# vision-agh/apse_uav

Measured on AMD Instinct MI355X. Metric: 4K UAV frames/sec (whole node), higher is better.
Workload: dtype f32

## Files before the change

apse_uav_amd/csrc/conv1x1_stream.hip:

```cpp
#include "apse_common.h"
#include <stdlib.h>
#include <type_traits>

typedef _Float16 f16x8 __attribute__((ext_vector_type(8)));
typedef unsigned s1_u32x4 __attribute__((ext_vector_type(4)));
__device__ __forceinline__ f32x16 s1_zero16() { return f32x16{0.f, 0.f, 0.f, 0.f, 0.f, 0.f, 0.f, 0.f, 0.f, 0.f, 0.f, 0.f, 0.f, 0.f, 0.f, 0.f}; }
__device__ __forceinline__ f32x16 s1_mfma16(bf16x8 a, bf16x8 b, f32x16 c) { return __builtin_amdgcn_mfma_f32_32x32x16_bf16(a, b, c, 0, 0, 0); }
__device__ __forceinline__ f32x16 s1_mfma16(f16x8 a, f16x8 b, f32x16 c) { return __builtin_amdgcn_mfma_f32_32x32x16_f16(a, b, c, 0, 0, 0); }

template <int PR, int KA, int NC = 128>
__global__ __launch_bounds__(256, 2) void conv1x1_stream(const ConvParams p, const int chunks_per_block) {
    constexpr int ESH = PR ? 1 : 2;
    constexpr int KSTEP = PR ? 64 : 32;
    constexpr int EPSLOT = 16 >> ESH;
    constexpr int NST = KA / KSTEP;
    constexpr int NJ = NC / 32;
    constexpr int CLD = 68;
    static_assert(NST >= 1 && KA % KSTEP == 0, "K must be a whole number of stages");
    extern __shared__ __attribute__((aligned(16))) char smem[];
    char* Ws = smem;
    float* Cw = reinterpret_cast<float*>(smem + 2 * NC * 128);

    const int tid = threadIdx.x, lane = tid & 63, wave = tid >> 6;
    const int fr = lane & 31, fh = lane >> 5;
    const int srow = tid >> 3, slot = tid & 7;
    const int M = p.M, N = p.Cout;
    const int m0 = blockIdx.x * 128 + wave * 32;
    const int chunks_total = N / NC;
    const int c_begin = blockIdx.y * chunks_per_block;
    const int c_end = (c_begin + chunks_per_block < chunks_total) ? c_begin + chunks_per_block : chunks_total;
    if (c_begin >= c_end) return;
    const int ohw = p.OH * p.OW;

    __amdgpu_buffer_rsrc_t xrsrc = __builtin_amdgcn_make_buffer_rsrc(const_cast<float*>(p.x), 0,
                                                                    (int)(((unsigned)(p.B * p.H * p.W) << p.cin_log2) << ESH), 0x00020000);
    f32x4 a[NST][4];
    {
        const int m = m0 + fr;
        unsigned base = 0xfffffff0u;
        if (m < M) {
            int pix = m;
            if (p.stride != 1) {
                const int b = m / ohw, rem = m - b * ohw, oy = rem / p.OW, ox = rem - oy * p.OW;
                pix = (b * p.H + oy * p.stride) * p.W + ox * p.stride;
            }
            base = ((unsigned)pix << p.cin_log2) << ESH;
        }
#pragma unroll
        for (int s = 0; s < NST; ++s)
#pragma unroll
            for (int c = 0; c < 4; ++c) {
                const unsigned off = (m < M) ? base + (unsigned)((s * KSTEP + (2 * c + fh) * EPSLOT) << ESH) : 0xfffffff0u;
                a[s][c] = __builtin_bit_cast(f32x4, __builtin_amdgcn_raw_buffer_load_b128(xrsrc, (int)off, 0, 0));
            }
    }

    const char* wbase = (PR ? reinterpret_cast<const char*>(p.w16) : reinterpret_cast<const char*>(p.w)) + ((size_t)(slot * EPSLOT) << ESH);
    const int G = (c_end - c_begin) * NST;
    f32x4 wr[NJ];
    auto w_fetch = [&](int g) {
        const int ch = c_begin + g / NST, s = g - (g / NST) * NST;
#pragma unroll
        for (int i = 0; i < NJ; ++i) {
            const size_t n = (size_t)ch * NC + srow + 32 * i;
            wr[i] = *reinterpret_cast<const f32x4*>(wbase + ((n * (size_t)p.KWCp + (size_t)s * KSTEP) << ESH));
        }
    };
    auto w_store = [&](int buf) {
#pragma unroll
        for (int i = 0; i < NJ; ++i) {
            const int row = srow + 32 * i;
            *reinterpret_cast<f32x4*>(Ws + buf * NC * 128 + row * 128 + ((slot ^ ((row >> 1) & 7)) << 4)) = wr[i];
        }
    };
    w_fetch(0);
    w_store(0);
    if (G > 1) w_fetch(1);
    __syncthreads();

    float* cw = Cw + wave * 32 * CLD;
    const int erow = lane >> 3, ecol = (lane & 7) * 8;
    constexpr unsigned ES = PR ? 2u : 4u, DEAD = 0x80000000u;
    unsigned yrow[4], rrow[4];
#pragma unroll
    for (int i = 0; i < 4; ++i) {
        const int m = m0 + erow + 8 * i;
        yrow[i] = m < M ? (unsigned)m * (unsigned)N * ES : DEAD;
        rrow[i] = yrow[i];
        if (p.res_mode == 2 && m < M) {
            const int b = m / ohw, rem = m - b * ohw, oy = rem / p.OW, ox = rem - oy * p.OW;
            rrow[i] = (unsigned)((b * (p.OH >> 1) + (oy >> 1)) * (p.OW >> 1) + (ox >> 1)) * (unsigned)N * ES;
        }
    }
    const unsigned res_rows = p.res_mode == 2 ? (unsigned)(p.B * (p.OH >> 1) * (p.OW >> 1)) : (unsigned)M;
    const __amdgpu_buffer_rsrc_t yrsrc = __builtin_amdgcn_make_buffer_rsrc(p.y, 0, (int)((unsigned)M * (unsigned)N * ES), 0x00020000);
    const __amdgpu_buffer_rsrc_t rrsrc = __builtin_amdgcn_make_buffer_rsrc(const_cast<float*>(p.res ? p.res : p.y), 0,
                                                                           (int)(p.res ? res_rows * (unsigned)N * ES : 0u), 0x00020000);
    int g = 0;
    for (int ch = c_begin; ch < c_end; ++ch) {
        f32x16 acc[NJ];
#pragma unroll
        for (int s = 0; s < NST; ++s, ++g) {
            const int buf = g & 1;
            if (g + 1 < G) w_store(buf ^ 1);
            if (g + 2 < G) w_fetch(g + 2);
            const char* Wb = Ws + buf * NC * 128;
#pragma unroll
            for (int c = 0; c < 4; ++c) {
                f32x4 bfr[NJ];
                const int ls = 2 * c + fh;
#pragma unroll
                for (int j = 0; j < NJ; ++j) {
                    const int row = j * 32 + fr;
                    bfr[j] = *reinterpret_cast<const f32x4*>(Wb + row * 128 + ((ls ^ ((row >> 1) & 7)) << 4));
                }
                if constexpr (PR != 0) {
                    typedef typename std::conditional<PR == 1, bf16x8, f16x8>::type op8;
#pragma unroll
                    for (int j = 0; j < NJ; ++j)
                        acc[j] = s1_mfma16(__builtin_bit_cast(op8, a[s][c]), __builtin_bit_cast(op8, bfr[j]), (s == 0 && c == 0) ? s1_zero16() : acc[j]);
                } else {
#pragma unroll
                    for (int k = 0; k < 4; ++k)
#pragma unroll
                        for (int j = 0; j < NJ; ++j)
                            acc[j] = __builtin_amdgcn_mfma_f32_32x32x2f32(a[s][c][k], bfr[j][k], (s == 0 && c == 0 && k == 0) ? s1_zero16() : acc[j], 0, 0, 0);
                }
            }
            __syncthreads();
        }
        const int n0 = ch * NC;
#pragma unroll
        for (int hh = 0; hh < NC / 64; ++hh) {
            const int nb = n0 + hh * 64 + ecol;
            constexpr int RV = PR ? 1 : 2;
            f32x4 rr[4][RV];
            if (p.res_mode != 0) {
#pragma unroll
                for (int i = 0; i < 4; ++i)
#pragma unroll
                    for (int q = 0; q < RV; ++q)
                        rr[i][q] = __builtin_bit_cast(f32x4, __builtin_amdgcn_raw_buffer_load_b128(rrsrc, (int)(rrow[i] + (unsigned)nb * ES + q * 16u), 0, 0));
            }
#pragma unroll
            for (int jj = 0; jj < 2; ++jj)
#pragma unroll
                for (int v = 0; v < 16; ++v)
                    cw[((v & 3) + 8 * (v >> 2) + 4 * fh) * CLD + jj * 32 + fr] = acc[2 * hh + jj][v];
            __builtin_amdgcn_wave_barrier();
            f32x4 b0 = {0.f, 0.f, 0.f, 0.f}, b1 = b0;
            if (p.bias) {
                b0 = *reinterpret_cast<const f32x4*>(p.bias + nb);
                b1 = *reinterpret_cast<const f32x4*>(p.bias + nb + 4);
            }
#pragma unroll
            for (int i = 0; i < 4; ++i) {
                const int r = erow + 8 * i;
                f32x4 v0 = *reinterpret_cast<const f32x4*>(cw + r * CLD + ecol) + b0;
                f32x4 v1 = *reinterpret_cast<const f32x4*>(cw + r * CLD + ecol + 4) + b1;
                if (p.res_mode != 0) {
                    if constexpr (PR == 0) { v0 += rr[i][0]; v1 += rr[i][RV - 1]; }
                    else {
                        const f32x4 raw = rr[i][0];
                        f32x4 x0, x1;
                        if constexpr (PR == 1) {
                            const unsigned q0 = __float_as_uint(raw[0]), q1 = __float_as_uint(raw[1]), q2 = __float_as_uint(raw[2]), q3 = __float_as_uint(raw[3]);
                            x0 = f32x4{__uint_as_float(q0 << 16), __uint_as_float(q0 & 0xffff0000u), __uint_as_float(q1 << 16), __uint_as_float(q1 & 0xffff0000u)};
                            x1 = f32x4{__uint_as_float(q2 << 16), __uint_as_float(q2 & 0xffff0000u), __uint_as_float(q3 << 16), __uint_as_float(q3 & 0xffff0000u)};
                        } else {
                            const f16x8 hv = __builtin_bit_cast(f16x8, raw);
                            x0 = f32x4{(float)hv[0], (float)hv[1], (float)hv[2], (float)hv[3]};
                            x1 = f32x4{(float)hv[4], (float)hv[5], (float)hv[6], (float)hv[7]};
                        }
                        v0 += x0; v1 += x1;
                    }
                }
                if (p.relu) {
#pragma unroll
                    for (int k = 0; k < 4; ++k) {
                        asm("v_max_f32 %0, 0, %1" : "=v"(v0[k]) : "v"(v0[k]));
                        asm("v_max_f32 %0, 0, %1" : "=v"(v1[k]) : "v"(v1[k]));
                    }
                }
                const int yoff = (int)(yrow[i] + (unsigned)nb * ES);
                if constexpr (PR == 0) {
                    __builtin_amdgcn_raw_buffer_store_b128(__builtin_bit_cast(s1_u32x4, v0), yrsrc, yoff, 0, APSE_NT ? 2 : 0);
                    __builtin_amdgcn_raw_buffer_store_b128(__builtin_bit_cast(s1_u32x4, v1), yrsrc, yoff + 16, 0, APSE_NT ? 2 : 0);
                } else if constexpr (PR == 1) {
                    bf16x8 o;
                    o[0] = (__bf16)v0[0]; o[1] = (__bf16)v0[1]; o[2] = (__bf16)v0[2]; o[3] = (__bf16)v0[3];
                    o[4] = (__bf16)v1[0]; o[5] = (__bf16)v1[1]; o[6] = (__bf16)v1[2]; o[7] = (__bf16)v1[3];
                    __builtin_amdgcn_raw_buffer_store_b128(__builtin_bit_cast(s1_u32x4, o), yrsrc, yoff, 0, APSE_NT ? 2 : 0);
                } else {
                    f16x8 o;
                    o[0] = (_Float16)v0[0]; o[1] = (_Float16)v0[1]; o[2] = (_Float16)v0[2]; o[3] = (_Float16)v0[3];
                    o[4] = (_Float16)v1[0]; o[5] = (_Float16)v1[1]; o[6] = (_Float16)v1[2]; o[7] = (_Float16)v1[3];
                    __builtin_amdgcn_raw_buffer_store_b128(__builtin_bit_cast(s1_u32x4, o), yrsrc, yoff, 0, APSE_NT ? 2 : 0);
                }
            }
            __builtin_amdgcn_wave_barrier();
        }
    }
}

bool apse_conv1x1_stream_ok(const ConvParams& p) {
    static const bool off = getenv("APSE_NO_STREAM1X1") != nullptr;
    if (off || p.no_stream) return false;
    const int K = 1 << p.cin_log2;
    if (p.KH != 1 || p.KW != 1 || p.pad != 0 || (p.stride != 1 && p.stride != 2)) return false;
    if (K != 64 && K != 128 && K != 256) return false;
    const bool nc64 = p.prec == 0 && K != 64;
    if (p.KWCp != K || (p.Cout & (nc64 ? 63 : 127)) != 0) return false;
    if (p.out_mode != 0 || p.y_coff != 0 || p.y_ld != p.Cout || p.splitk != 1 || p.m_count || p.tile_cnt) return false;
    if (p.res_mode != 0 && p.res_mode != 1 && p.res_mode != 2) return false;
    if ((((size_t)p.B * p.H * p.W) << p.cin_log2) * (p.prec ? 2 : 4) >= 0xfffffff0ull) return false;
    if (((size_t)p.M + 128) * (size_t)p.Cout * (p.prec ? 2 : 4) >= 0x70000000ull) return false;
    if (p.y_st != p.prec || (p.res_mode != 0 && p.res_st != p.prec)) return false;
    if (p.prec == 0) {
        static const bool no128 = getenv("APSE_NO_STREAM_F32K128") != nullptr, no256 = getenv("APSE_NO_STREAM_F32K256") != nullptr;
        return p.x_st == 0 && p.w != nullptr &&
               (K == 64 || (K == 128 && !no128) || (K == 256 && !no256 && p.stride == 1 && (size_t)p.OH * p.OW >= 32768));
    }
    return p.x_st == p.prec && p.w16 != nullptr;
}

template <int PR, int KA, int NC = 128>
static int launch_stream(const ConvParams& p, hipStream_t s, hipEvent_t ev0, hipEvent_t ev1) {
    const size_t lds = 2 * NC * 128 + 4 * 32 * 68 * sizeof(float);
    static bool attr_done = false;
    if (!attr_done) {
        hipFuncSetAttribute(reinterpret_cast<const void*>(&conv1x1_stream<PR, KA, NC>), hipFuncAttributeMaxDynamicSharedMemorySize, (int)lds);
        attr_done = true;
    }
    const int mblocks = (p.M + 127) / 128, chunks = p.Cout / NC;
    static const int want = getenv("APSE_STREAM_BLOCKS") ? atoi(getenv("APSE_STREAM_BLOCKS")) : 256;
    int ysplit = 1;
    while (mblocks * ysplit < want && ysplit < chunks) ysplit *= 2;
    if (ysplit > chunks) ysplit = chunks;
    const int per = (chunks + ysplit - 1) / ysplit;
    if (ev0) hipEventRecord(ev0, s);
    hipLaunchKernelGGL((conv1x1_stream<PR, KA, NC>), dim3(mblocks, (chunks + per - 1) / per), dim3(256), lds, s, p, per);
    if (ev1) hipEventRecord(ev1, s);
    return hipGetLastError() == hipSuccess ? APSE_OK : APSE_E_HIP;
}

int apse_launch_conv1x1_stream(const ConvParams& p, hipStream_t s, hipEvent_t ev0, hipEvent_t ev1) {
    const int K = 1 << p.cin_log2;
    if (p.prec == 0) return K == 64 ? launch_stream<0, 64>(p, s, ev0, ev1) : (K == 128 ? launch_stream<0, 128, 64>(p, s, ev0, ev1) : launch_stream<0, 256, 64>(p, s, ev0, ev1));
    if (p.prec == 1) {
        if (K == 64) return launch_stream<1, 64>(p, s, ev0, ev1);
        if (K == 128) return launch_stream<1, 128>(p, s, ev0, ev1);
        return launch_stream<1, 256>(p, s, ev0, ev1);
    }
    if (K == 64) return launch_stream<2, 64>(p, s, ev0, ev1);
    if (K == 128) return launch_stream<2, 128>(p, s, ev0, ev1);
    return launch_stream<2, 256>(p, s, ev0, ev1);
}
```

Baseline: 204.2.

## Stream activations progressively and prefetch bias/residual ahead of conv1x1 epilogue

For f32 kernels with many K stages, activation loads are spread across the first chunk's K loop (three stages ahead) instead of all being issued up front, and weights are double-buffered in two register sets with sched barriers to order loads, MFMAs and LDS stores. The first output chunk is peeled so this prologue logic runs only once. Bias and residual loads move to buffer loads, and for non-progressive K>64 variants they are issued before the last K stage so they overlap the MFMAs. This raises register pressure, since an extra weight set and prefetched residual tiles are held, which may hurt occupancy under the 256x2 launch bounds.

```diff
diff --git a/apse_uav_amd/csrc/conv1x1_stream.hip b/apse_uav_amd/csrc/conv1x1_stream.hip
--- a/apse_uav_amd/csrc/conv1x1_stream.hip
+++ b/apse_uav_amd/csrc/conv1x1_stream.hip
@@ -15,8 +15,15 @@
     constexpr int EPSLOT = 16 >> ESH;
     constexpr int NST = KA / KSTEP;
     constexpr int NJ = NC / 32;
+    constexpr int NH = NC / 64;
     constexpr int CLD = 68;
+    constexpr bool PROG = PR == 0 && NST >= 8;
+    constexpr bool PEEL = KA != 64;
+    constexpr bool RAHEAD = PEEL && !PROG;
+    constexpr int AD = PROG ? 3 : NST;
+    constexpr int WSETS = PROG ? 2 : 1;
     static_assert(NST >= 1 && KA % KSTEP == 0, "K must be a whole number of stages");
+    static_assert(!PROG || NST % 2 == 0, "PROG takes the LDS buffer and the register set from the parity of s");
     extern __shared__ __attribute__((aligned(16))) char smem[];
     char* Ws = smem;
     float* Cw = reinterpret_cast<float*>(smem + 2 * NC * 128);
@@ -35,47 +42,59 @@
     __amdgpu_buffer_rsrc_t xrsrc = __builtin_amdgcn_make_buffer_rsrc(const_cast<float*>(p.x), 0,
                                                                     (int)(((unsigned)(p.B * p.H * p.W) << p.cin_log2) << ESH), 0x00020000);
     f32x4 a[NST][4];
-    {
-        const int m = m0 + fr;
-        unsigned base = 0xfffffff0u;
-        if (m < M) {
-            int pix = m;
-            if (p.stride != 1) {
-                const int b = m / ohw, rem = m - b * ohw, oy = rem / p.OW, ox = rem - oy * p.OW;
-                pix = (b * p.H + oy * p.stride) * p.W + ox * p.stride;
-            }
-            base = ((unsigned)pix << p.cin_log2) << ESH;
-        }
-#pragma unroll
-        for (int s = 0; s < NST; ++s)
-#pragma unroll
-            for (int c = 0; c < 4; ++c) {
-                const unsigned off = (m < M) ? base + (unsigned)((s * KSTEP + (2 * c + fh) * EPSLOT) << ESH) : 0xfffffff0u;
-                a[s][c] = __builtin_bit_cast(f32x4, __builtin_amdgcn_raw_buffer_load_b128(xrsrc, (int)off, 0, 0));
-            }
+    const int am = m0 + fr;
+    unsigned abase = 0xfffffff0u;
+    if (am < M) {
+        int pix = am;
+        if (p.stride != 1) {
+            const int b = am / ohw, rem = am - b * ohw, oy = rem / p.OW, ox = rem - oy * p.OW;
+            pix = (b * p.H + oy * p.stride) * p.W + ox * p.stride;
+        }
+        abase = ((unsigned)pix << p.cin_log2) << ESH;
+    }
+    auto a_fetch = [&](int s) {
+#pragma unroll
+        for (int c = 0; c < 4; ++c) {
+            const unsigned off = (am < M) ? abase + (unsigned)((s * KSTEP + (2 * c + fh) * EPSLOT) << ESH) : 0xfffffff0u;
+            a[s][c] = __builtin_bit_cast(f32x4, __builtin_amdgcn_raw_buffer_load_b128(xrsrc, (int)off, 0, 0));
+        }
+    };
+    if constexpr (!PROG) {
+#pragma unroll
+        for (int s = 0; s < NST; ++s) a_fetch(s);
     }
 
     const char* wbase = (PR ? reinterpret_cast<const char*>(p.w16) : reinterpret_cast<const char*>(p.w)) + ((size_t)(slot * EPSLOT) << ESH);
     const int G = (c_end - c_begin) * NST;
-    f32x4 wr[NJ];
-    auto w_fetch = [&](int g) {
+    f32x4 wr[WSETS][NJ];
+    auto w_fetch = [&](int g, int set) {
         const int ch = c_begin + g / NST, s = g - (g / NST) * NST;
 #pragma unroll
         for (int i = 0; i < NJ; ++i) {
             const size_t n = (size_t)ch * NC + srow + 32 * i;
-            wr[i] = *reinterpret_cast<const f32x4*>(wbase + ((n * (size_t)p.KWCp + (size_t)s * KSTEP) << ESH));
-        }
-    };
-    auto w_store = [&](int buf) {
+            wr[set][i] = *reinterpret_cast<const f32x4*>(wbase + ((n * (size_t)p.KWCp + (size_t)s * KSTEP) << ESH));
+        }
+    };
+    auto w_store = [&](int buf, int set) {
 #pragma unroll
         for (int i = 0; i < NJ; ++i) {
             const int row = srow + 32 * i;
-            *reinterpret_cast<f32x4*>(Ws + buf * NC * 128 + row * 128 + ((slot ^ ((row >> 1) & 7)) << 4)) = wr[i];
-        }
-    };
-    w_fetch(0);
-    w_store(0);
-    if (G > 1) w_fetch(1);
+            *reinterpret_cast<f32x4*>(Ws + buf * NC * 128 + row * 128 + ((slot ^ ((row >> 1) & 7)) << 4)) = wr[set][i];
+        }
+    };
+    if constexpr (PROG) {
+        w_fetch(0, 0);
+        w_fetch(1, 1);
+        __builtin_amdgcn_sched_barrier(0);
+#pragma unroll
+        for (int s = 0; s < AD; ++s) a_fetch(s);
+        __builtin_amdgcn_sched_barrier(0);
+        w_store(0, 0);
+    } else {
+        w_fetch(0, 0);
+        w_store(0, 0);
+        if (G > 1) w_fetch(1, 0);
+    }
     __syncthreads();
 
     float* cw = Cw + wave * 32 * CLD;
@@ -96,14 +115,46 @@
     const __amdgpu_buffer_rsrc_t yrsrc = __builtin_amdgcn_make_buffer_rsrc(p.y, 0, (int)((unsigned)M * (unsigned)N * ES), 0x00020000);
     const __amdgpu_buffer_rsrc_t rrsrc = __builtin_amdgcn_make_buffer_rsrc(const_cast<float*>(p.res ? p.res : p.y), 0,
                                                                            (int)(p.res ? res_rows * (unsigned)N * ES : 0u), 0x00020000);
-    int g = 0;
-    for (int ch = c_begin; ch < c_end; ++ch) {
-        f32x16 acc[NJ];
-#pragma unroll
-        for (int s = 0; s < NST; ++s, ++g) {
-            const int buf = g & 1;
-            if (g + 1 < G) w_store(buf ^ 1);
-            if (g + 2 < G) w_fetch(g + 2);
+    const __amdgpu_buffer_rsrc_t brsrc = __builtin_amdgcn_make_buffer_rsrc(const_cast<float*>(p.bias ? p.bias : p.y), 0,
+                                                                           (int)(p.bias ? (unsigned)N * 4u : 0u), 0x00020000);
+    constexpr int RV = PR ? 1 : 2;
+    f32x4 rr[NH][4][RV], bb[NH][2];
+    auto b_fetch = [&](int ch, int hh) {
+        const int nb = ch * NC + hh * 64 + ecol;
+        bb[hh][0] = __builtin_bit_cast(f32x4, __builtin_amdgcn_raw_buffer_load_b128(brsrc, nb * 4, 0, 0));
+        bb[hh][1] = __builtin_bit_cast(f32x4, __builtin_amdgcn_raw_buffer_load_b128(brsrc, nb * 4 + 16, 0, 0));
+    };
+    auto r_fetch = [&](int ch, int hh, f32x4 (&dst)[4][RV]) {
+        const int nb = ch * NC + hh * 64 + ecol;
+#pragma unroll
+        for (int i = 0; i < 4; ++i)
+#pragma unroll
+            for (int q = 0; q < RV; ++q)
+                dst[i][q] = __builtin_bit_cast(f32x4, __builtin_amdgcn_raw_buffer_load_b128(rrsrc, (int)(rrow[i] + (unsigned)nb * ES + q * 16u), 0, 0));
+    };
+
+    auto k_stages = [&](auto first_tag, f32x16 (&acc)[NJ], const int ch, const int gbase) {
+        constexpr bool FIRST = decltype(first_tag)::value;
+#pragma unroll
+        for (int s = 0; s < NST; ++s) {
+            const int g = gbase + s;
+            const int buf = PROG ? (s & 1) : (g & 1);
+            if (RAHEAD && s == NST - 1) {
+                b_fetch(ch, 0);
+                r_fetch(ch, 0, rr[0]);
+                __builtin_amdgcn_sched_barrier(0);
+            }
+            if constexpr (PROG) {
+                w_fetch((FIRST && s + 2 < NST) || g + 2 < G ? g + 2 : G - 1, s & 1);
+                if (FIRST && s + AD < NST) {
+                    __builtin_amdgcn_sched_barrier(0);
+                    a_fetch(s + AD);
+                }
+            } else {
+                if (g + 1 < G) w_store(buf ^ 1, 0);
+                if (g + 2 < G) w_fetch(g + 2, 0);
+            }
+            if constexpr (PROG) __builtin_amdgcn_sched_barrier(0);
             const char* Wb = Ws + buf * NC * 128;
 #pragma unroll
             for (int c = 0; c < 4; ++c) {
@@ -127,21 +178,31 @@
                             acc[j] = __builtin_amdgcn_mfma_f32_32x32x2f32(a[s][c][k], bfr[j][k], (s == 0 && c == 0 && k == 0) ? s1_zero16() : acc[j], 0, 0, 0);
                 }
             }
+            if constexpr (PROG) {
+                __builtin_amdgcn_sched_barrier(0);
+                if ((FIRST && s + 1 < NST) || g + 1 < G) w_store(buf ^ 1, (s + 1) & 1);
+            }
             __syncthreads();
         }
+    };
+
+    auto epilogue = [&](f32x16 (&acc)[NJ], const int ch) {
         const int n0 = ch * NC;
 #pragma unroll
-        for (int hh = 0; hh < NC / 64; ++hh) {
+        for (int hh = 0; hh < NH; ++hh) {
             const int nb = n0 + hh * 64 + ecol;
-            constexpr int RV = PR ? 1 : 2;
-            f32x4 rr[4][RV];
-            if (p.res_mode != 0) {
-#pragma unroll
-                for (int i = 0; i < 4; ++i)
-#pragma unroll
-                    for (int q = 0; q < RV; ++q)
-                        rr[i][q] = __builtin_bit_cast(f32x4, __builtin_amdgcn_raw_buffer_load_b128(rrsrc, (int)(rrow[i] + (unsigned)nb * ES + q * 16u), 0, 0));
-            }
+            f32x4 rl[4][RV];
+            if constexpr (!RAHEAD) {
+                if constexpr (PEEL) b_fetch(ch, hh);
+                if (p.res_mode != 0) r_fetch(ch, hh, rl);
+            } else if (hh + 1 < NH) {
+                b_fetch(ch, hh + 1);
+                r_fetch(ch, hh + 1, rr[hh + 1]);
+            }
+            auto res_row = [&](int i, int q) -> f32x4 {
+                if constexpr (RAHEAD) return rr[hh][i][q];
+                else return rl[i][q];
+            };
 #pragma unroll
             for (int jj = 0; jj < 2; ++jj)
 #pragma unroll
@@ -149,7 +210,10 @@
                     cw[((v & 3) + 8 * (v >> 2) + 4 * fh) * CLD + jj * 32 + fr] = acc[2 * hh + jj][v];
             __builtin_amdgcn_wave_barrier();
             f32x4 b0 = {0.f, 0.f, 0.f, 0.f}, b1 = b0;
-            if (p.bias) {
+            if constexpr (PEEL) {
+                b0 = bb[hh][0];
+                b1 = bb[hh][1];
+            } else if (p.bias) {
                 b0 = *reinterpret_cast<const f32x4*>(p.bias + nb);
                 b1 = *reinterpret_cast<const f32x4*>(p.bias + nb + 4);
             }
@@ -159,9 +223,9 @@
                 f32x4 v0 = *reinterpret_cast<const f32x4*>(cw + r * CLD + ecol) + b0;
                 f32x4 v1 = *reinterpret_cast<const f32x4*>(cw + r * CLD + ecol + 4) + b1;
                 if (p.res_mode != 0) {
-                    if constexpr (PR == 0) { v0 += rr[i][0]; v1 += rr[i][RV - 1]; }
+                    if constexpr (PR == 0) { v0 += res_row(i, 0); v1 += res_row(i, RV - 1); }
                     else {
-                        const f32x4 raw = rr[i][0];
+                        const f32x4 raw = res_row(i, 0);
                         f32x4 x0, x1;
                         if constexpr (PR == 1) {
                             const unsigned q0 = __float_as_uint(raw[0]), q1 = __float_as_uint(raw[1]), q2 = __float_as_uint(raw[2]), q3 = __float_as_uint(raw[3]);
@@ -200,6 +264,18 @@
             }
             __builtin_amdgcn_wave_barrier();
         }
+    };
+
+    if constexpr (PEEL) {
+        f32x16 acc[NJ];
+        k_stages(std::integral_constant<bool, PROG>{}, acc, c_begin, 0);
+        epilogue(acc, c_begin);
+    }
+    int g0 = PEEL ? NST : 0;
+    for (int ch = c_begin + (PEEL ? 1 : 0); ch < c_end; ++ch, g0 += NST) {
+        f32x16 acc[NJ];
+        k_stages(std::false_type{}, acc, ch, g0);
+        epilogue(acc, ch);
     }
 }
 
```

Result: no change. 204.4 (median of 6 runs) (+0.1%).
